# syun88/VLA-from-FastVLM

Measured on AMD Instinct MI355X. Metric: policy steps/sec (img+prompt->action) FastVLM-0.5B bs=64, higher is better.
Workload: dtype bf16; 1 GPU; fastvlm-0.5b select_action: letterbox 336^2->1024^2, FastViT-HD, projector, Qwen2 decoder (text-only, reference-literal: 64-token prompt), last-token pool, action head; batch_per_gpu=64, global_batch=64, seq_len=64, image=336, parallelism=replicas x1 (no collective on the inference path), tower_microbatch=0, stream_overlap=True, llm_precision=split-bf16 (hi+lo) operands, fp32 attention

## Files before the change

include/fastvla_hip_testops.h:

```cpp
#ifndef FASTVLA_HIP_TESTOPS_H
#define FASTVLA_HIP_TESTOPS_H

#include "fastvla_hip.h"

#ifdef __cplusplus
extern "C" {
#endif

enum fv_gemm_epilogue {
  FV_EPI_BIAS = 0,
  FV_EPI_BIAS_GELU = 1,
  FV_EPI_LS_RES = 2,
  FV_EPI_RES_F32 = 3,
  FV_EPI_SWIGLU = 4,
  FV_EPI_F32 = 5,
  FV_EPI_SWIGLU_SPLIT = 7,
  FV_EPI_SWIGLU_F16 = 8,
  FV_EPI_GELU_GRAD = 9,
  FV_EPI_MUL_AUX = 10,
  FV_EPI_F16 = 11,
  FV_EPI_MUL_GELUP = 12
};
int fv_op_gemm(const void* A, int lda, const void* W, int M, int N, int K, const float* bias, const float* scale,
               const void* res, int ldr, void* out, int ldo, int epilogue, fv_stream s);
// ... 14 lines not shown
int fv_op_stem_mfma(const void* pix, const void* wp, const float* bias, void* y, int B, int S, int Cout, fv_stream s);
int fv_op_stem_fused(const void* pix, const void* wp, const float* b1, const float* w2, const float* b2, void* y, int B,
                     int S, int Cout, fv_stream s);
int fv_op_stem_fused_images(const void* img, int dtype, int B, int C, int Hin, int Win, float pad_value, int resize_with_padding, const void* wp,
                            const float* b1, const float* w2, const float* b2, void* y, int S, int Cout, fv_stream s);
int fv_op_layernorm_rows(const void* x, const float* w, const float* b, void* y, int rows, int C, float eps,
                         fv_stream s);
int fv_op_attention(const void* q, const void* k, const void* v, int ldq, int ldk, int ldv, void* out, int ldo, int B,
                    int T, int heads, int kv_heads, int D, int causal, const int32_t* lens, float scale, fv_stream s);
int fv_op_attention_bf16(const void* q, const void* k, const void* v, int ldq, int ldk, int ldv, void* out, int ldo, int B, int T, int heads, int kv_heads, int D,
                         int causal, const int32_t* lens, int len_add, float scale, fv_stream s);
int fv_op_tower_attention_bwd(const void* qkv, int ld, const void* dO, int lddo, void* dqkv, int ldd, float* stats, int B, int T, int heads, float scale, fv_stream s);
int fv_op_rmsnorm(const float* x, const float* w, void* y_bf16, int rows, int H, float eps, fv_stream s);
int fv_op_rope(void* qkv, int ld, int rows, int T, int heads, int kv_heads, int D, float theta, fv_stream s);
int fv_op_attention_bwd(const float* qkv, int ld, const float* dO, float* dqkv, void* out_bf16_scratch, float* stat_scratch, int B, int T,
                        int heads, int kv_heads, int D, const int32_t* lens, float theta, fv_stream s);
int fv_op_attention_bwd_routes(const float* qkv, int ld, const float* dO, int lddo, float* dqkv, void* out_bf16, int ldo, float* stat, float* part, int B, int T,
                               int heads, int kv_heads, int D, const int32_t* lens, int len_add, float theta, int use_split, fv_stream s);
int fv_op_attention_f32(void* qkv, int ld, void* out, int ldo, int B, int T, int heads, int kv_heads, int D, const int32_t* lens, int len_add,
                        const void* rope_table, const void* pre, int ldp, int Np, float* lse, int lo8, int use_split, fv_stream s);
int fv_op_rmsnorm_forms(const float* x, const float* w, void* y, void* y_lo, int ldy, int rows, int H, float eps, int f16, unsigned* sat, int lo8, fv_stream s);
int fv_op_embed_gather(const int32_t* ids, const void* table, const float* img_tokens, float* x, int B, int T, int Ni, int H, int vocab, fv_stream s);
int fv_op_pool_norm(const float* x, const int32_t* lens, const float* w, float* pooled, int B, int Ttot, int Ni, int H, float eps, int mode, fv_stream s);
int fv_op_rmsnorm_bwd(const float* x, const float* w, const float* dy, const float* dres, float* dx, float* dw, float* scratch, int rows,
                      int H, float eps, fv_stream s);

int fv_op_se_gelu(const void* x, const float* w1, const float* b1, const float* w2, const float* b2, void* y,
                  float* scratch, int B, int P, int C, int R, fv_stream s);

int fv_op_dwconv_mfma(const void* x, const void* ttab, const float* bias, void* y, int B, int H, int W, int C, int k, int gelu,
                      fv_stream s);
int fv_op_dwconv_s2_mfma(const void* x, const void* ttab, const float* bias, void* y, int B, int H, int W, int C, int gelu,
                         fv_stream s);
int fv_op_dwconv_pair(const void* x, const void* t3, const float* b3, const void* t7, const float* b7, void* y1, void* y2, int B,
                      int H, int W, int C, fv_stream s);
int fv_op_convffn(const void* x, const void* w1, const float* b1, const void* w2p, const float* b2, const float* ls,
                  const void* res, void* out, int M, int C, fv_stream s);

int fv_op_convffn32(const void* x, const void* wq, const float* b1, const float* b2, const float* ls, const void* res, void* out,
                    int M, int C, fv_stream s);
int fv_op_convffn32_stash(const void* x, const void* wq, const float* b1, const float* b2, const float* ls, const void* res, void* out,
                          int M, int C, void* stash_y, fv_stream s);
int fv_op_gemm_f16_gelup(const void* A, int lda, const void* W, int M, int N, int K, const void* aux, int ldaux, void* out, int ldo, void* h_out, fv_stream s);
int fv_op_dw_wgrad(const void* x, const void* dy, float* dw, float* db, float* scratch, size_t scratch_floats, int B, int H, int W, int C, int k, int stride, int mult, fv_stream s);
int fv_op_dw_dgrad(const void* dy, const float* w, const void* res, void* dx, int B, int Hi, int Wi, int Ci, int k, int stride, int mult, int round_w, unsigned* sat,
                   fv_stream s);
int fv_op_dw_dgrad_mfma(const void* dy, const void* ttab16, const void* res, void* dx, int B, int H, int W, int C, int k, unsigned* sat, fv_stream s);
int fv_op_convffn32_split(const void* x, const void* wq, const float* b1, const float* b2, const float* ls, const void* res, void* out,
                          int M, int C, float* part, size_t part_bytes, fv_stream s);

int fv_op_lora_direct_scratch_floats(int R, int rank, int max_cols, size_t* out_floats);
int fv_op_lora_direct(int kind, int part_mask, int rank, int Np, int K, int qd, int kd, const int64_t* a_off, const int64_t* b_off, const void* dY, const void* X,
                      int xkind, int ldx, int lo_off, int R, const float* lora, float* lora_grads, float scale, float* scratch, size_t scratch_floats, fv_stream s);


int fv_op_chunk_loss(const float* a, const float* t, const uint8_t* pad, float* g, float* partial, size_t partial_floats, float* loss, float* metrics,
                     int64_t n, int A, int kind, float beta, float loss_scale, fv_stream s);

int fv_op_chunk_loss_weighted(const float* a, const float* t, const uint8_t* pad, const float* dim_w, const float* step_w, float* g, float* partial,
                              size_t partial_floats, float* loss, float* metrics, int64_t n, int A, int K, int kind, float beta, float loss_scale, fv_stream s);

int fv_op_head_loss_backward(int feat, int ds, int da, int hid, int fus, int time_dim, const float* P, const float* actions, const float* targets,
                             const uint8_t* pad, int kind, float beta, int chunk, int B, const void* saved, float* loss, float* metrics, float* G,
                             float* scratch, size_t scratch_floats, float* d_pooled, fv_stream s);
int fv_op_head_loss_backward_draws(int feat, int ds, int da, int hid, int fus, int time_dim, int draws, const float* P, const float* actions, const float* targets,
                                   const uint8_t* pad, const float* dim_w, const float* step_w, int kind, float beta, int chunk, int B, const void* saved, float* loss,
// ... 17 lines not shown
```

vla-from-fastvlm_amd/csrc/kernels.h:

```cpp
#pragma once
#include <hip/hip_runtime.h>
#include <stdint.h>

#include "../../include/fastvla_hip.h"
#include "../../include/fastvla_hip_testops.h"
#include "common.h"

namespace fv {

struct GemmArgs {
  const bf16_t* A; int lda;
  const bf16_t* W;
  int M, N, K;
  const float* bias;
  const float* scale;
  const void* res; int ldr;
  void* out; int ldo;
  int epi;
  int ksplit = 0;
  int f16 = 0;
  float* splitk_ws = nullptr;
  size_t splitk_bytes = 0;
  int lo_off = 0;
  int no_tail = 0;
// ... 17 lines not shown
void convffn32_pack(const float* w1, const float* w2, float* out, int C);
int launch_convffn32(const bf16_t* x, const bf16_t* wq, const float* b1, const float* b2, const float* ls,
                     const bf16_t* res, bf16_t* out, int M, int C, int hidden, hipStream_t s, float* part = nullptr, size_t part_bytes = 0,
                     bf16_t* stash_y = nullptr);
bool convffn32_stash_supported(int M, int C);

int launch_letterbox(const void* img, int dtype, int B, int C, int Hin, int Win, int S, float pad_value, int letterbox,
                     bf16_t* pix, hipStream_t s);
int launch_letterbox_norm(const void* img, int dtype, int B, int C, int Hin, int Win, int S, float pad_value, int letterbox, const float* mean3,
                          const float* std3, int range_heuristic, unsigned* vmax_scratch, bf16_t* pix, hipStream_t s);
int launch_augment_draw(const fv_augment_config* cfg, const void* img, int dtype, int B, int C, int Hin, int Win, uint64_t seed, uint64_t offset,
                        uint64_t sample_base, fv_augment_sample* table, hipStream_t s);
int launch_letterbox_augmented(const void* img, int dtype, int B, int C, int Hin, int Win, int S, float pad_value, int letterbox,
                               const fv_augment_sample* table, float value_max, bf16_t* pix, hipStream_t s);
int launch_stem_conv(const bf16_t* pix, const float* w, const float* bias, bf16_t* y, int B, int S, int Cout,
                     hipStream_t s);
void stem_mfma_pack(const float* w27, float* out, int Cout);
int launch_stem_mfma(const bf16_t* pix, const bf16_t* wp, const float* bias, bf16_t* y, int B, int S, int Cout, hipStream_t s);
bool stem_fused_supported(int S, int C0);
int launch_stem_fused(const bf16_t* pix, const bf16_t* wp, const float* b1, const float* w2, const float* b2, bf16_t* y, int B,
                      int S, int C0, hipStream_t s);
int launch_stem_fused_lb(const void* img, int dtype, int B, int C, int Hin, int Win, float pad_value, int letterbox, const bf16_t* wp,
                         const float* b1, const float* w2, const float* b2, bf16_t* y, int S, int C0, hipStream_t s);
int launch_dwconv(const bf16_t* x, const float* w, const float* bias, bf16_t* y, int B, int H, int W, int C, int k,
                  int stride, int mult, int gelu, hipStream_t s);
bool dwconv_mfma_supported(int W, int C, int k, int stride, int mult);
size_t dwconv_toeplitz_elems(int C, int k);
void dwconv_toeplitz_pack(const float* w_tapmajor, float* out, int C, int k);
size_t dwconv_s2_toeplitz_elems(int C);
void dwconv_s2_toeplitz_pack(const float* w_tapmajor, float* out, int C);
bool dwconv_s2_mfma_supported(int H, int W, int C, int k, int stride, int mult);
int launch_dwconv_s2_mfma(const bf16_t* x, const bf16_t* ttab, const float* bias, bf16_t* y, int B, int H, int W, int C, int gelu,
                          hipStream_t s);
bool dwconv_pair_supported(int B, int H, int W, int C);
int launch_dwconv_pair(const bf16_t* x, const bf16_t* t3, const float* b3, const bf16_t* t7, const float* b7, bf16_t* y1, bf16_t* y2,
                       int B, int H, int W, int C, hipStream_t s);
int launch_dwconv_mfma(const bf16_t* x, const bf16_t* ttab, const float* bias, bf16_t* y, int B, int H, int W, int C, int k,
                       int gelu, hipStream_t s);
int launch_layernorm_rows(const bf16_t* x, const float* w, const float* b, bf16_t* y, int rows, int C, float eps,
                          hipStream_t s);
int launch_se_gelu(const bf16_t* x, const float* w1, const float* b1, const float* w2, const float* b2, bf16_t* y,
                   float* scratch, int B, int P, int C, int R, hipStream_t s);
int launch_attention(const bf16_t* q, const bf16_t* k, const bf16_t* v, int ldq, int ldk, int ldv, bf16_t* out,
                     int ldo, int B, int T, int heads, int kv_heads, int D, int causal, const int32_t* lens,
                     int len_add, float scale, hipStream_t s, const unsigned* skip = nullptr);

int launch_embed_gather(const int32_t* ids, const bf16_t* table, const float* img_tokens, float* x, int B, int T,
                        int Ni, int H, int vocab, hipStream_t s, const unsigned* skip = nullptr);
int launch_rmsnorm(const float* x, const float* w, bf16_t* y, bf16_t* y_lo, int ldy, int rows, int H, float eps, hipStream_t s,
                   int f16 = 0, unsigned* sat = nullptr,
                   int lo8 = 0, const unsigned* skip = nullptr);
int launch_bf16_to_f16(bf16_t* p, size_t n, float scale, hipStream_t s, unsigned* maxbits = nullptr);
int launch_bf16_to_w8(const bf16_t* w, void* w8, size_t rows, int K, hipStream_t s, unsigned* maxbits = nullptr);
int launch_rope_f32(float* qkv, const float2* table, int ld, int rows, int T, int heads, int kv_heads, int D, hipStream_t s, const unsigned* skip = nullptr);
int launch_attention_f32(float* qkv, int ld, bf16_t* out_hi, bf16_t* out_lo, int ldo, int B, int T, int heads,
                         int kv_heads, int D, const int32_t* lens, int len_add, float scale, hipStream_t s, const float2* rope = nullptr,
                         const float* pre = nullptr, int ldp = 0, int Np = 0,
                         float* lse = nullptr,
                         int lo8 = 0,
                         void* split_scratch = nullptr,
                         const unsigned* skip = nullptr);
constexpr int FV_ATTN_SPLIT_MIN_T = 128;
int launch_rope(bf16_t* qkv, const float2* table, int ld, int rows, int T, int heads, int kv_heads, int D,
                hipStream_t s, const unsigned* skip = nullptr);
void rope_table_host(float* cos_sin_pairs, int T, int D, float theta);
int launch_pool_norm(const float* x, const int32_t* lens, const float* w, float* pooled, int B, int Ttot, int Ni,
// ... 211 lines not shown
```

vla-from-fastvlm_amd/csrc/ops_api.hip:

```cpp
#include <cmath>
#include <vector>

#include "kernels.h"

extern "C" {

int fv_op_gemm(const void* A, int lda, const void* W, int M, int N, int K, const float* bias, const float* scale,
               const void* res, int ldr, void* out, int ldo, int epilogue, fv_stream s) {
  fv::GemmArgs g{static_cast<const bf16_t*>(A), lda, static_cast<const bf16_t*>(W), M, N, K, bias, scale, res, ldr, out, ldo, epilogue};
  return fv::launch_gemm(g, static_cast<hipStream_t>(s));
}
int fv_op_gemm_ksplit(const void* A, int lda, const void* W, int M, int N, int K, const float* bias, const void* res, int ldr,
                      void* out, int ldo, int epilogue, fv_stream s) {
  fv::GemmArgs g{static_cast<const bf16_t*>(A), lda, static_cast<const bf16_t*>(W), M, N, K, bias, nullptr, res, ldr, out, ldo, epilogue};
  g.ksplit = true;
  return fv::launch_gemm(g, static_cast<hipStream_t>(s));
}
int fv_op_gemm_splitk(const void* A, int lda, const void* W, int M, int N, int K, const float* bias, const void* res, int ldr,
                      void* out, int ldo, int epilogue, int ksplit, void* ws, size_t ws_bytes, fv_stream s) {
  fv::GemmArgs g{static_cast<const bf16_t*>(A), lda, static_cast<const bf16_t*>(W), M, N, K, bias, nullptr, res, ldr, out, ldo, epilogue};
  g.ksplit = ksplit != 0;
  g.splitk_ws = static_cast<float*>(ws);
  g.splitk_bytes = ws_bytes;
  return fv::launch_gemm(g, static_cast<hipStream_t>(s));
// ... 160 lines not shown
}

int fv_op_rmsnorm_forms(const float* x, const float* w, void* y, void* y_lo, int ldy, int rows, int H, float eps, int f16, unsigned* sat, int lo8, fv_stream s) {
  return fv::launch_rmsnorm(x, w, static_cast<bf16_t*>(y), static_cast<bf16_t*>(y_lo), ldy, rows, H, eps, static_cast<hipStream_t>(s), f16, sat, lo8);
}

int fv_op_embed_gather(const int32_t* ids, const void* table, const float* img_tokens, float* x, int B, int T, int Ni, int H, int vocab, fv_stream s) {
  return fv::launch_embed_gather(ids, static_cast<const bf16_t*>(table), img_tokens, x, B, T, Ni, H, vocab, static_cast<hipStream_t>(s));
}

int fv_op_pool_norm(const float* x, const int32_t* lens, const float* w, float* pooled, int B, int Ttot, int Ni, int H, float eps, int mode, fv_stream s) {
  return fv::launch_pool_norm(x, lens, w, pooled, B, Ttot, Ni, H, eps, mode, static_cast<hipStream_t>(s));
}

int fv_op_rmsnorm_bwd(const float* x, const float* w, const float* dy, const float* dres, float* dx, float* dw, float* scratch, int rows,
                      int H, float eps, fv_stream s) {
  return fv::launch_rmsnorm_bwd(x, w, dy, dres, dx, dw, scratch, rows, H, eps, static_cast<hipStream_t>(s));
}

int fv_op_se_gelu(const void* x, const float* w1, const float* b1, const float* w2, const float* b2, void* y,
                  float* scratch, int B, int P, int C, int R, fv_stream s) {
  return fv::launch_se_gelu(static_cast<const bf16_t*>(x), w1, b1, w2, b2, static_cast<bf16_t*>(y), scratch, B, P, C, R, static_cast<hipStream_t>(s));
}

int fv_op_dwconv_mfma(const void* x, const void* ttab, const float* bias, void* y, int B, int H, int W, int C, int k, int gelu,
                      fv_stream s) {
  return fv::launch_dwconv_mfma(static_cast<const bf16_t*>(x), static_cast<const bf16_t*>(ttab), bias, static_cast<bf16_t*>(y), B, H, W, C, k,
                                gelu, static_cast<hipStream_t>(s));
}
int fv_op_dwconv_s2_mfma(const void* x, const void* ttab, const float* bias, void* y, int B, int H, int W, int C, int gelu, fv_stream s) {
  return fv::launch_dwconv_s2_mfma(static_cast<const bf16_t*>(x), static_cast<const bf16_t*>(ttab), bias, static_cast<bf16_t*>(y), B, H, W, C,
                                   gelu, static_cast<hipStream_t>(s));
}
int fv_op_dwconv_pair(const void* x, const void* t3, const float* b3, const void* t7, const float* b7, void* y1, void* y2, int B,
                      int H, int W, int C, fv_stream s) {
  return fv::launch_dwconv_pair(static_cast<const bf16_t*>(x), static_cast<const bf16_t*>(t3), b3, static_cast<const bf16_t*>(t7), b7,
                                static_cast<bf16_t*>(y1), static_cast<bf16_t*>(y2), B, H, W, C, static_cast<hipStream_t>(s));
}

int fv_op_convffn(const void* x, const void* w1, const float* b1, const void* w2p, const float* b2, const float* ls,
                  const void* res, void* out, int M, int C, fv_stream s) {
  return fv::launch_convffn(static_cast<const bf16_t*>(x), static_cast<const bf16_t*>(w1), b1, static_cast<const bf16_t*>(w2p), b2, ls,
                            static_cast<const bf16_t*>(res), static_cast<bf16_t*>(out), M, C, 4 * C, static_cast<hipStream_t>(s));
}

int fv_op_convffn32(const void* x, const void* wq, const float* b1, const float* b2, const float* ls, const void* res, void* out,
                    int M, int C, fv_stream s) {
  return fv::launch_convffn32(static_cast<const bf16_t*>(x), static_cast<const bf16_t*>(wq), b1, b2, ls, static_cast<const bf16_t*>(res),
                              static_cast<bf16_t*>(out), M, C, 4 * C, static_cast<hipStream_t>(s));
}

int fv_op_convffn32_stash(const void* x, const void* wq, const float* b1, const float* b2, const float* ls, const void* res, void* out,
                          int M, int C, void* stash_y, fv_stream s) {
  if (!stash_y) return fv_fail(FV_ERR_ARG, "fv_op_convffn32_stash: null stash");
  return fv::launch_convffn32(static_cast<const bf16_t*>(x), static_cast<const bf16_t*>(wq), b1, b2, ls, static_cast<const bf16_t*>(res),
                              static_cast<bf16_t*>(out), M, C, 4 * C, static_cast<hipStream_t>(s), nullptr, 0, static_cast<bf16_t*>(stash_y));
}
int fv_op_gemm_f16_gelup(const void* A, int lda, const void* W, int M, int N, int K, const void* aux, int ldaux, void* out, int ldo, void* h_out, fv_stream s) {
  fv::GemmArgs g{static_cast<const bf16_t*>(A), lda, static_cast<const bf16_t*>(W), M, N, K, nullptr, nullptr, aux, ldaux, out, ldo, FV_EPI_MUL_GELUP};
  g.f16 = 1;
  g.stash = h_out;
  return fv::launch_gemm(g, static_cast<hipStream_t>(s));
}

int fv_op_dw_wgrad(const void* x, const void* dy, float* dw, float* db, float* scratch, size_t scratch_floats, int B, int H, int W, int C, int k, int stride, int mult, fv_stream s) {
  const int pad = k / 2, Ho = (H + 2 * pad - k) / stride + 1, Wo = (W + 2 * pad - k) / stride + 1;
// ... 142 lines not shown
```

vla-from-fastvlm_amd/csrc/tower_kernels.hip:

```cpp
#include "kernels.h"
#include "letterbox.h"
#include <cstdlib>

namespace fv {
namespace {

__device__ __forceinline__ uint2 lb_pixel(const LbParams& p, int b, int y, int x) {
  float v[3] = {p.pad, p.pad, p.pad};
  const int dx = x - p.pl, dy = y - p.pt;
  if (dx >= 0 && dx < p.rw && dy >= 0 && dy < p.rh) {
    const float sx = lb_src(dx, p.sw);
    const int x0 = min((int)sx, p.Win - 1), x1 = min(x0 + 1, p.Win - 1);
    const float wx = lb_frac(sx, x0);
    const float sy = lb_src(dy, p.sh);
    const int y0 = min((int)sy, p.Hin - 1), y1 = min(y0 + 1, p.Hin - 1);
    const float wy = lb_frac(sy, y0);
    const int nc = p.C >= 3 ? 3 : 1;
    for (int c = 0; c < nc; ++c) {
      const size_t plane = ((size_t)b * p.C + c) * p.Hin * p.Win;
      const float t0 = lb_lerp(lb_fetch(p, plane, y0, x0), lb_fetch(p, plane, y0, x1), wx);
      const float t1 = lb_lerp(lb_fetch(p, plane, y1, x0), lb_fetch(p, plane, y1, x1), wx);
      v[c] = lb_lerp(t0, t1, wy);
    }
    if (nc == 1) v[1] = v[2] = v[0];
// ... 743 lines not shown
        uint2 u;
        u.x = pack_bf2(g[0].x, g[0].y);
        u.y = pack_bf2(g[1].x, g[1].y);
        *reinterpret_cast<uint2*>(sX + ((rg * 4 + jr) * 4 + q) * OC + ((co ^ sig) << 3)) = u;
      }
  }
  __syncthreads();
  {
    const int cg = tid & 7, quad = (tid >> 3) & 3, row = tid >> 5;
    const int sig = (row >> 1) & 1;
    uint2 r[8];
#pragma unroll
    for (int e = 0; e < 8; ++e) r[e] = *reinterpret_cast<const uint2*>(sX + (row * 4 + quad) * OC + (((cg * 8 + e) ^ sig) << 3));
    const int oy = tyb * TH + row, ox0 = tx * TW + quad * 4;
    if (oy < Ho) {
      bf16_t* yp = y + (((size_t)b * Ho + oy) * Wo + ox0) * (2 * C) + 2 * c0 + cg * 8;
#pragma unroll
      for (int j = 0; j < 4; ++j) {
        if (ox0 + j < Wo) {
          uint4 o;
          const uint32_t sel = (j & 1) ? 0x07060302u : 0x05040100u;
#define FV_PX(A, B) __builtin_amdgcn_perm((j & 2) ? r[B].y : r[B].x, (j & 2) ? r[A].y : r[A].x, sel)
          o.x = FV_PX(0, 1); o.y = FV_PX(2, 3); o.z = FV_PX(4, 5); o.w = FV_PX(6, 7);
#undef FV_PX
          *reinterpret_cast<uint4*>(yp + (size_t)j * (2 * C)) = o;
        }
      }
    }
  }
  __syncthreads();
  tx = txn; tyb = tybn; b = bn;
  }
}

#ifndef DW_MARCH_OCC
#define DW_MARCH_OCC 2
#endif
typedef __attribute__((ext_vector_type(4))) _Float16 f16x4_t;
__device__ __forceinline__ _Float16 f2h_ovf(float v) { return (_Float16)(fabsf(v) > FV_F16_MAX ? copysignf(__builtin_inff(), v) : v); }
template <bool GRAD> struct MarchAux { typedef const float* type; };
template <> struct MarchAux<true> { typedef unsigned* type; };
template <bool GRAD> using march_aux_t = typename MarchAux<GRAD>::type;
template <int K, bool GRAD = false>
__global__ __launch_bounds__(256, DW_MARCH_OCC) void dwconv_march_kernel(const bf16_t* __restrict__ x, const bf16_t* __restrict__ ttab,
                                                               march_aux_t<GRAD> __restrict__ aux, bf16_t* __restrict__ y,
                                                               int H, int W, int C, int gelu, int tiles_x, int nslices, const bf16_t* __restrict__ res = nullptr) {
  constexpr int TW = 32, PAD = K / 2, IW = TW + K - 1;
  constexpr int NQ = (IW + 3) / 4, NM = (K + 3 + 3) / 4;
  constexpr int RS = NQ * 256 + 64, RSO = 8 * 256 + 64;
  constexpr int T_BYTES = 2 * K * NM * 512;
#if DW_MARCH_OCC >= 3
  __shared__ __attribute__((aligned(16))) char smem[16 * RS];
#else
  __shared__ __attribute__((aligned(16))) char smem[16 * RS + 8 * RSO];
#endif
  extern __shared__ __attribute__((aligned(16))) char smem_lo[];
  static_assert(!GRAD || DW_MARCH_OCC < 3, "the GRAD instances keep an output tile of their own");
  char* sX = smem;

  const int tid = threadIdx.x, lane = tid & 63, wid = tid >> 6;
  int bid = xcd_remap(blockIdx.x, gridDim.x);
  const int slice = bid % nslices; bid /= nslices;
  const int tx = bid % tiles_x;
  const long b = bid / tiles_x;
  const int c0 = slice * 32;
  const int gg = wid & 1, rg = wid >> 1;
// ... 735 lines not shown
size_t dwconv_toeplitz_elems(int C, int k) { return (size_t)(C / 16) * k * ((k + 6) / 4) * 256; }
void dwconv_toeplitz_pack(const float* w_tapmajor, float* out, int C, int k) {
  const int NM = (k + 6) / 4;
  for (int g = 0; g < C / 16; ++g)
    for (int ky = 0; ky < k; ++ky)
      for (int m = 0; m < NM; ++m)
        for (int bch = 0; bch < 16; ++bch)
          for (int i = 0; i < 4; ++i)
            for (int kk = 0; kk < 4; ++kk) {
              const int kx = 4 * m + kk - i;
              out[((((size_t)(g * k + ky) * NM + m) * 16 + bch) * 4 + i) * 4 + kk] =
                  (kx >= 0 && kx < k) ? w_tapmajor[(size_t)(ky * k + kx) * C + g * 16 + bch] : 0.0f;
            }
}
size_t dwconv_s2_toeplitz_elems(int C) { return (size_t)(C / 16) * 2 * 7 * 4 * 256; }
void dwconv_s2_toeplitz_pack(const float* w_tapmajor, float* out, int C) {
  for (int g = 0; g < C / 16; ++g)
    for (int e = 0; e < 2; ++e)
      for (int ky = 0; ky < 7; ++ky)
        for (int m = 0; m < 4; ++m)
          for (int bch = 0; bch < 16; ++bch)
            for (int i = 0; i < 4; ++i)
              for (int kk = 0; kk < 4; ++kk) {
                const int kx = 4 * m + kk - 2 * i;
                out[(((((size_t)(g * 2 + e) * 7 + ky) * 4 + m) * 16 + bch) * 4 + i) * 4 + kk] =
                    (kx >= 0 && kx < 7) ? w_tapmajor[(size_t)(ky * 7 + kx) * (2 * C) + 2 * (g * 16 + bch) + e] : 0.0f;
              }
}
bool dwconv_s2_mfma_supported(int H, int W, int C, int k, int stride, int mult) {
  return k == 7 && stride == 2 && mult == 2 && C % 32 == 0 && H % 2 == 0 && W % 2 == 0 && W >= 16;
}
int launch_dwconv_s2_mfma(const bf16_t* x, const bf16_t* ttab, const float* bias, bf16_t* y, int B, int H, int W, int C, int gelu,
                          hipStream_t s) {
  if (!x || !ttab || !bias || !y) return fv_fail(FV_ERR_ARG, "dwconv_s2_mfma: null pointer");
  if (B <= 0 || H <= 0 || !dwconv_s2_mfma_supported(H, W, C, 7, 2, 2)) return fv_fail(FV_ERR_UNSUPPORTED, "dwconv_s2_mfma: unsupported shape H=%d W=%d C=%d", H, W, C);
  const int Ho = H / 2, Wo = W / 2;
  const int tiles_x = (Wo + 15) / 16, tiles_y = (Ho + 7) / 8, nsl = C / 32;
  const long nblk = (long)B * tiles_x * tiles_y * nsl;
  if (nblk > 0x7fffffffL) return fv_fail(FV_ERR_ARG, "dwconv_s2_mfma: grid too large");
  static int cus = 0;
  if (!cus) {
    int dev = 0;
    hipDeviceProp_t prop;
    cus = (hipGetDevice(&dev) == hipSuccess && hipGetDeviceProperties(&prop, dev) == hipSuccess && prop.multiProcessorCount > 0) ? prop.multiProcessorCount : 256;
  }
  const long tiles = nblk / nsl, tpx = (tiles + 7) / 8;
  long chains = (2L * cus / 8) / nsl;
  if (chains < 1) chains = 1;
  if (chains > tpx) chains = tpx;
  hipLaunchKernelGGL(dwconv_s2_mfma_kernel, dim3((unsigned)(8 * chains * nsl)), dim3(256), 0, s, x, ttab, bias, y, H, W, C, Ho, Wo, gelu, tiles_x, tiles_y, nsl, B);
  FV_HIP_CHECK(hipGetLastError());
  return FV_OK;
}

bool dwconv_mfma_supported(int W, int C, int k, int stride, int mult) {
  return stride == 1 && mult == 1 && (k == 3 || k == 7) && W >= 16 && C % 32 == 0;
}

int launch_dwconv_mfma(const bf16_t* x, const bf16_t* ttab, const float* bias, bf16_t* y, int B, int H, int W, int C, int k,
                       int gelu, hipStream_t s) {
  if (!x || !ttab || !bias || !y) return fv_fail(FV_ERR_ARG, "dwconv_mfma: null pointer");
  if (B <= 0 || H <= 0 || !dwconv_mfma_supported(W, C, k, 1, 1)) return fv_fail(FV_ERR_UNSUPPORTED, "dwconv_mfma: unsupported shape W=%d C=%d k=%d", W, C, k);
#ifndef DW_TH7
#define DW_TH7 8
#endif
  const int th = (k == 7 && H >= 32) ? DW_TH7 : 8;
  const int tiles_x = (W + 31) / 32, tiles_y = (H + th - 1) / th, nsl = C / 32;
  const long nblk = (long)B * tiles_x * tiles_y * nsl;
  if (nblk > 0x7fffffffL) return fv_fail(FV_ERR_ARG, "dwconv_mfma: grid too large");
#ifndef DW_NO_MARCH
  if (k == 7 && H >= 16) {
    const long nstrips = (long)B * tiles_x * nsl;
// ... 165 lines not shown
```

vla-from-fastvlm_amd/fastvla_hip/_lib.py:

```python
from __future__ import annotations

import ctypes as C
import os
from pathlib import Path

FV_MAX_STAGES = 8
FV_F32, FV_BF16, FV_U8, FV_I32 = 0, 1, 2, 3
EPI_BIAS, EPI_BIAS_GELU, EPI_LS_RES, EPI_RES_F32, EPI_SWIGLU, EPI_F32 = range(6)
EPI_SWIGLU_SPLIT = 7
EPI_SWIGLU_F16 = 8


class FastVLAHipError(RuntimeError):
    status = 0


class ModelDesc(C.Structure):
    _fields_ = [
        ("llm_hidden", C.c_int32), ("llm_layers", C.c_int32), ("llm_heads", C.c_int32), ("llm_kv_heads", C.c_int32),
        ("llm_head_dim", C.c_int32), ("llm_inter", C.c_int32), ("llm_vocab", C.c_int32),
        ("rope_theta", C.c_float), ("rms_eps", C.c_float),
        ("tower_stages", C.c_int32),
        ("tower_layers", C.c_int32 * FV_MAX_STAGES), ("tower_dims", C.c_int32 * FV_MAX_STAGES),
        ("tower_is_attn", C.c_int32 * FV_MAX_STAGES),
# ... 164 lines not shown
    "fv_train_tower_backward": (_i, [_vp, _vp, _vp, _i, _vp, C.c_size_t, _vp, BUCKET_CB, _vp, _vp]),
    "fv_train_tower_read_unit": (_i, [_vp, _i, _i, _vp, C.c_size_t, _vp, _vp]),
    "fv_train_tower_unit": (_i, [_vp, _i, _vp, _vp, _f, _i, _vp, C.c_size_t, _vp, _vp, _vp, _vp]),
    "fv_profile": (_i, [_vp, _i]),
    "fv_profile_read": (_i, [_vp, C.POINTER(ProfileEntry), C.POINTER(GemmProfile), _i, C.POINTER(_i)]),
    "fv_adamw_clip_step": (_i, [_vp, _vp, _vp, _vp, _vp, _i64, C.POINTER(AdamWHParams), _i64, _vp, _vp]),
    "fv_adamw_groups_create": (_i, [_vp, C.POINTER(AdamWGroup), _i, _i64, C.POINTER(_vp)]),
    "fv_adamw_groups_destroy": (_i, [_vp, _vp]),
    "fv_adamw_clip_step_groups": (_i, [_vp, _vp, _vp, _vp, _vp, _i64, C.POINTER(AdamWHParams), _vp, _i64, _vp, _vp, _vp]),
    "fv_adamw_clip_step_ema": (_i, [_vp, _vp, _vp, _vp, _vp, _vp, _f, _i64, C.POINTER(AdamWHParams), _vp, _i64, _vp, _vp, _vp]),
}

OPS_SIGNATURES = {
    "fv_op_gemm": (_i, [_vp, _i, _vp, _i, _i, _i, _vp, _vp, _vp, _i, _vp, _i, _i, _vp]),
    "fv_op_gemm_f16": (_i, [_vp, _i, _vp, _i, _i, _i, _vp, _vp, _i, _vp, _i, _i, _vp, C.c_size_t, _vp]),
    "fv_op_gemm_lo8": (_i, [_vp, _i, _vp, _vp, _i, _i, _i, _vp, _vp, _i, _vp, _i, _i, _vp, C.c_size_t, _vp]),
    "fv_op_lo8_pack": (_i, [_vp, _vp, _i, _vp, _vp, _i, _i, _i, _vp]),
    "fv_op_gemm_ksplit": (_i, [_vp, _i, _vp, _i, _i, _i, _vp, _vp, _i, _vp, _i, _i, _vp]),
    "fv_op_gemm_tn": (_i, [_vp, _i, _vp, _i, _i, _i, _i, _i, _vp, _vp, _i, _vp, C.c_size_t, _vp]),
    "fv_op_gemm_splitk": (_i, [_vp, _i, _vp, _i, _i, _i, _vp, _vp, _i, _vp, _i, _i, _i, _vp, C.c_size_t, _vp]),
    "fv_op_dwconv": (_i, [_vp, _vp, _vp, _vp, _i, _i, _i, _i, _i, _i, _i, _i, _vp]),
    "fv_op_stem_conv": (_i, [_vp, _vp, _vp, _vp, _i, _i, _i, _vp]),
    "fv_op_stem_mfma": (_i, [_vp, _vp, _vp, _vp, _i, _i, _i, _vp]),
    "fv_op_stem_fused": (_i, [_vp, _vp, _vp, _vp, _vp, _vp, _i, _i, _i, _vp]),
    "fv_op_stem_fused_images": (_i, [_vp, _i, _i, _i, _i, _i, _f, _i, _vp, _vp, _vp, _vp, _vp, _i, _i, _vp]),
    "fv_op_layernorm_rows": (_i, [_vp, _vp, _vp, _vp, _i, _i, _f, _vp]),
    "fv_op_attention": (_i, [_vp, _vp, _vp, _i, _i, _i, _vp, _i, _i, _i, _i, _i, _i, _i, _vp, _f, _vp]),
    "fv_op_attention_bf16": (_i, [_vp, _vp, _vp, _i, _i, _i, _vp, _i, _i, _i, _i, _i, _i, _i, _vp, _i, _f, _vp]),
    "fv_op_tower_attention_bwd": (_i, [_vp, _i, _vp, _i, _vp, _i, _vp, _i, _i, _i, _f, _vp]),
    "fv_op_rmsnorm": (_i, [_vp, _vp, _vp, _i, _i, _f, _vp]),
    "fv_op_rope": (_i, [_vp, _i, _i, _i, _i, _i, _i, _f, _vp]),
    "fv_op_dwconv_mfma": (_i, [_vp, _vp, _vp, _vp, _i, _i, _i, _i, _i, _i, _vp]),
    "fv_op_dwconv_s2_mfma": (_i, [_vp, _vp, _vp, _vp, _i, _i, _i, _i, _i, _vp]),
    "fv_op_dwconv_pair": (_i, [_vp, _vp, _vp, _vp, _vp, _vp, _vp, _i, _i, _i, _i, _vp]),
    "fv_op_convffn": (_i, [_vp, _vp, _vp, _vp, _vp, _vp, _vp, _vp, _i, _i, _vp]),
    "fv_op_convffn32": (_i, [_vp, _vp, _vp, _vp, _vp, _vp, _vp, _i, _i, _vp]),
    "fv_op_convffn32_stash": (_i, [_vp, _vp, _vp, _vp, _vp, _vp, _vp, _i, _i, _vp, _vp]),
    "fv_op_gemm_f16_gelup": (_i, [_vp, _i, _vp, _i, _i, _i, _vp, _i, _vp, _i, _vp, _vp]),
    "fv_op_dw_wgrad": (_i, [_vp, _vp, _vp, _vp, _vp, C.c_size_t, _i, _i, _i, _i, _i, _i, _i, _vp]),
    "fv_op_dw_dgrad": (_i, [_vp, _vp, _vp, _vp, _i, _i, _i, _i, _i, _i, _i, _i, _vp, _vp]),
    "fv_op_dw_dgrad_mfma": (_i, [_vp, _vp, _vp, _vp, _i, _i, _i, _i, _i, _vp, _vp]),
    "fv_op_convffn32_split": (_i, [_vp, _vp, _vp, _vp, _vp, _vp, _vp, _i, _i, _vp, C.c_size_t, _vp]),
    "fv_op_lora_direct_scratch_floats": (_i, [_i, _i, _i, C.POINTER(C.c_size_t)]),
    "fv_op_lora_direct": (_i, [_i, _i, _i, _i, _i, _i, _i, _vp, _vp, _vp, _vp, _i, _i, _i, _i, _vp, _vp, _f, _vp, C.c_size_t, _vp]),
    "fv_op_attention_bwd": (_i, [_vp, _i, _vp, _vp, _vp, _vp, _i, _i, _i, _i, _i, _vp, _f, _vp]),
    "fv_op_attention_bwd_routes": (_i, [_vp, _i, _vp, _i, _vp, _vp, _i, _vp, _vp, _i, _i, _i, _i, _i, _vp, _i, _f, _i, _vp]),
    "fv_op_rmsnorm_bwd": (_i, [_vp, _vp, _vp, _vp, _vp, _vp, _vp, _i, _i, _f, _vp]),
    "fv_op_attention_f32": (_i, [_vp, _i, _vp, _i, _i, _i, _i, _i, _i, _vp, _i, _vp, _vp, _i, _i, _vp, _i, _i, _vp]),
    "fv_op_rmsnorm_forms": (_i, [_vp, _vp, _vp, _vp, _i, _i, _i, _f, _i, _vp, _i, _vp]),
    "fv_op_embed_gather": (_i, [_vp, _vp, _vp, _vp, _i, _i, _i, _i, _i, _vp]),
    "fv_op_pool_norm": (_i, [_vp, _vp, _vp, _vp, _i, _i, _i, _i, _f, _i, _vp]),
    "fv_op_chunk_loss": (_i, [_vp, _vp, _vp, _vp, _vp, C.c_size_t, _vp, _vp, _i64, _i, _i, _f, _f, _vp]),
    "fv_op_chunk_loss_weighted": (_i, [_vp, _vp, _vp, _vp, _vp, _vp, _vp, C.c_size_t, _vp, _vp, _i64, _i, _i, _i, _f, _f, _vp]),
    "fv_op_head_loss_backward": (_i, [_i, _i, _i, _i, _i, _i, _vp, _vp, _vp, _vp, _i, _f, _i, _i, _vp, _vp, _vp, _vp, _vp, C.c_size_t, _vp, _vp]),
    "fv_op_head_loss_backward_draws": (_i, [_i, _i, _i, _i, _i, _i, _i, _vp, _vp, _vp, _vp, _vp, _vp, _i, _f, _i, _i, _vp, _vp, _vp, _vp, _vp, C.c_size_t, _vp, _vp]),
    "fv_op_flow_vjp": (_i, [_i, _i, _i, _i, _i, _i, _vp, _vp, _vp, _vp, _i, _vp, _f, _vp, _vp, _vp, _vp, C.c_size_t, _vp]),
    "fv_op_flow_vjp_prefix": (_i, [_i, _i, _i, _i, _i, _i, _i, _vp, _vp, _vp, _vp, _i, _vp, _f, _vp, _vp, _vp, _vp, C.c_size_t, _vp]),
    "fv_op_flow_select": (_i, [_vp, _i, _i, _i, _i, _vp, _i, _vp, _vp, _i, _vp, _vp, _vp, _vp, _vp, _vp, _vp, _vp, _vp]),
    "fv_op_head_saved_cat_offset": (_i, [_i, _i, _i, _i, _i, _i, _i, _i, _i, C.POINTER(C.c_size_t)]),
    "fv_op_se_gelu": (_i, [_vp, _vp, _vp, _vp, _vp, _vp, _vp, _i, _i, _i, _i, _vp]),
}

_LIB = None
_OPS = None


# ... 82 lines not shown
```

Before: 21.85 steps/s.

## Add row-marching stride-2 depthwise conv kernel with LDS ring buffer

Adds a new stride-2 7x7 depthwise MFMA kernel in which each block marches down the full image height for one x-tile and channel slice. Input rows are held in a 21-row LDS ring, and global fetches for the next group are prefetched into registers while the current group computes. By default it replaces the per-tile kernel whenever Ho>=16, and a route argument allows forcing either path. The intent is to stop reloading the halo rows that overlapping tiles share and to overlap loads with compute. The cost is a much smaller grid (no tiles_y dimension) and a large dynamic LDS footprint, which may reduce parallelism.

```diff
diff --git a/include/fastvla_hip_testops.h b/include/fastvla_hip_testops.h
--- a/include/fastvla_hip_testops.h
+++ b/include/fastvla_hip_testops.h
@@ -70,6 +70,8 @@
                       fv_stream s);
 int fv_op_dwconv_s2_mfma(const void* x, const void* ttab, const float* bias, void* y, int B, int H, int W, int C, int gelu,
                          fv_stream s);
+int fv_op_dwconv_s2_route(const void* x, const void* ttab, const float* bias, void* y, int B, int H, int W, int C, int gelu, int route,
+                          fv_stream s);
 int fv_op_dwconv_pair(const void* x, const void* t3, const float* b3, const void* t7, const float* b7, void* y1, void* y2, int B,
                       int H, int W, int C, fv_stream s);
 int fv_op_convffn(const void* x, const void* w1, const float* b1, const void* w2p, const float* b2, const float* ls,
diff --git a/vla-from-fastvlm_amd/csrc/kernels.h b/vla-from-fastvlm_amd/csrc/kernels.h
--- a/vla-from-fastvlm_amd/csrc/kernels.h
+++ b/vla-from-fastvlm_amd/csrc/kernels.h
@@ -73,6 +73,8 @@
 bool dwconv_s2_mfma_supported(int H, int W, int C, int k, int stride, int mult);
 int launch_dwconv_s2_mfma(const bf16_t* x, const bf16_t* ttab, const float* bias, bf16_t* y, int B, int H, int W, int C, int gelu,
                           hipStream_t s);
+int launch_dwconv_s2_mfma_route(const bf16_t* x, const bf16_t* ttab, const float* bias, bf16_t* y, int B, int H, int W, int C, int gelu,
+                                int route, hipStream_t s);
 bool dwconv_pair_supported(int B, int H, int W, int C);
 int launch_dwconv_pair(const bf16_t* x, const bf16_t* t3, const float* b3, const bf16_t* t7, const float* b7, bf16_t* y1, bf16_t* y2,
                        int B, int H, int W, int C, hipStream_t s);
diff --git a/vla-from-fastvlm_amd/csrc/ops_api.hip b/vla-from-fastvlm_amd/csrc/ops_api.hip
--- a/vla-from-fastvlm_amd/csrc/ops_api.hip
+++ b/vla-from-fastvlm_amd/csrc/ops_api.hip
@@ -216,6 +216,10 @@
   return fv::launch_dwconv_s2_mfma(static_cast<const bf16_t*>(x), static_cast<const bf16_t*>(ttab), bias, static_cast<bf16_t*>(y), B, H, W, C,
                                    gelu, static_cast<hipStream_t>(s));
 }
+int fv_op_dwconv_s2_route(const void* x, const void* ttab, const float* bias, void* y, int B, int H, int W, int C, int gelu, int route, fv_stream s) {
+  return fv::launch_dwconv_s2_mfma_route(static_cast<const bf16_t*>(x), static_cast<const bf16_t*>(ttab), bias, static_cast<bf16_t*>(y), B, H, W, C,
+                                         gelu, route, static_cast<hipStream_t>(s));
+}
 int fv_op_dwconv_pair(const void* x, const void* t3, const float* b3, const void* t7, const float* b7, void* y1, void* y2, int B,
                       int H, int W, int C, fv_stream s) {
   return fv::launch_dwconv_pair(static_cast<const bf16_t*>(x), static_cast<const bf16_t*>(t3), b3, static_cast<const bf16_t*>(t7), b7,
diff --git a/vla-from-fastvlm_amd/csrc/tower_kernels.hip b/vla-from-fastvlm_amd/csrc/tower_kernels.hip
--- a/vla-from-fastvlm_amd/csrc/tower_kernels.hip
+++ b/vla-from-fastvlm_amd/csrc/tower_kernels.hip
@@ -799,6 +799,169 @@
   tx = txn; tyb = tybn; b = bn;
   }
 }
+
+__global__ __launch_bounds__(256, 2) void dwconv_s2_march_kernel(const bf16_t* __restrict__ x, const bf16_t* __restrict__ ttab,
+                                                                  const float* __restrict__ bias, bf16_t* __restrict__ y, int H,
+                                                                  int W, int C, int Ho, int Wo, int gelu, int tiles_x, int nslices) {
+  constexpr int K = 7, TW = 16, PAD = 3, IW = 2 * TW + K - 2;
+  constexpr int NQ = (IW + 3) / 4, NM = 4;
+  constexpr int RS = NQ * 256 + 64;
+  constexpr int RING = 21, UR = 16, PR = RING - UR;
+  constexpr int OC = 512 + 16;
+  constexpr int UTASK = UR * NQ * 4, PTASK = PR * NQ * 4, TPT = (UTASK + 255) / 256;
+  extern __shared__ __attribute__((aligned(16))) char smem_s2m[];
+  char* sX = smem_s2m;
+  char* sO = smem_s2m + RING * RS;
+  const int tid = threadIdx.x, lane = tid & 63, wid = tid >> 6;
+  int bid = xcd_remap(blockIdx.x, gridDim.x);
+  const int slice = bid % nslices; bid /= nslices;
+  const int tx = bid % tiles_x;
+  const int b = bid / tiles_x;
+  const int c0 = slice * 32;
+  const int gg = wid & 1, eo = wid >> 1;
+  const int bch = lane >> 2, jr = lane & 3;
+  const int ng = (Ho + 7) >> 3;
+
+  s16x4 afr[K][NM];
+  {
+    const char* tsrc = reinterpret_cast<const char*>(ttab) + (size_t)(slice * 2 + gg) * (2 * K * NM * 512) + (size_t)eo * (K * NM * 512) + lane * 8;
+#pragma unroll
+    for (int ky = 0; ky < K; ++ky)
+#pragma unroll
+      for (int m = 0; m < NM; ++m) afr[ky][m] = __builtin_bit_cast(s16x4, *reinterpret_cast<const uint2*>(tsrc + (ky * NM + m) * 512));
+  }
+  uint4 px[TPT][4];
+  int trow[TPT], tcol[TPT], toff[TPT];
+  uint32_t tcell[TPT];
+#pragma unroll
+  for (int tt = 0; tt < TPT; ++tt) {
+    const int task = min(tid + 256 * tt, UTASK - 1);
+    const int cg = task & 3, quad = (task >> 2) % NQ, row = (task >> 2) / NQ;
+    trow[tt] = row;
+    tcol[tt] = quad * 4;
+    toff[tt] = (row * W + quad * 4) * C + cg * 8;
+    tcell[tt] = (uint32_t)(quad * 256 + cg * 64) | (uint32_t)((((quad & 3) << 1) | (cg >> 1)) << 3);
+  }
+  const int ix0 = 2 * tx * TW - PAD;
+  auto fetch = [&](int r0, int ntask) {
+    const bf16_t* org = x + ((long)b * H * W + (long)r0 * W + ix0) * C + c0;
+#pragma unroll
+    for (int tt = 0; tt < TPT; ++tt) {
+      const bool rok = tid + 256 * tt < ntask && (unsigned)(r0 + trow[tt]) < (unsigned)H;
+#pragma unroll
+      for (int j = 0; j < 4; ++j)
+        px[tt][j] = (rok && (unsigned)(ix0 + tcol[tt] + j) < (unsigned)W) ? *reinterpret_cast<const uint4*>(org + toff[tt] + j * C)
+                                                                         : make_uint4(0, 0, 0, 0);
+    }
+  };
+  auto stage = [&](int p0, int ntask) {
+#pragma unroll
+    for (int tt = 0; tt < TPT; ++tt) {
+      if (tid + 256 * tt < ntask) {
+        const uint32_t d[4][4] = {{px[tt][0].x, px[tt][0].y, px[tt][0].z, px[tt][0].w}, {px[tt][1].x, px[tt][1].y, px[tt][1].z, px[tt][1].w},
+                                  {px[tt][2].x, px[tt][2].y, px[tt][2].z, px[tt][2].w}, {px[tt][3].x, px[tt][3].y, px[tt][3].z, px[tt][3].w}};
+        int pr = p0 + trow[tt];
+        pr -= pr >= RING ? RING : 0;
+        const uint32_t dst = (uint32_t)(pr * RS) + tcell[tt];
+#pragma unroll
+        for (int dd = 0; dd < 4; ++dd) {
+          uint2 ev, od;
+          ev.x = __builtin_amdgcn_perm(d[1][dd], d[0][dd], 0x05040100u);
+          ev.y = __builtin_amdgcn_perm(d[3][dd], d[2][dd], 0x05040100u);
+          od.x = __builtin_amdgcn_perm(d[1][dd], d[0][dd], 0x07060302u);
+          od.y = __builtin_amdgcn_perm(d[3][dd], d[2][dd], 0x07060302u);
+          *reinterpret_cast<uint2*>(sX + (dst ^ (uint32_t)((2 * dd) * 8))) = ev;
+          *reinterpret_cast<uint2*>(sX + (dst ^ (uint32_t)((2 * dd + 1) * 8))) = od;
+        }
+      }
+    }
+  };
+  uint32_t sw[4];
+#pragma unroll
+  for (int v = 0; v < 4; ++v) sw[v] = (uint32_t)(((gg * 16 + bch) ^ ((v << 1) | gg)) << 3);
+  const int co = 2 * (gg * 16 + bch) + eo;
+  const float bv = bias[2 * c0 + co];
+
+  fetch(-PAD, PTASK);
+  stage(0, PTASK);
+  fetch(PR - PAD, UTASK);
+  stage(PR, UTASK);
+  if (ng > 1) fetch(UR + PR - PAD, UTASK);
+  int gb = 0;
+  for (int g = 0; g < ng; ++g) {
+    __syncthreads();
+    f32x4 acc[2][4];
+#pragma unroll
+    for (int rg = 0; rg < 2; ++rg)
+#pragma unroll
+      for (int q = 0; q < 4; ++q) acc[rg][q] = f32x4{0.f, 0.f, 0.f, 0.f};
+    int lb = gb + 2 * jr;
+    lb -= lb >= RING ? RING : 0;
+#pragma unroll
+    for (int ky = 0; ky < K; ++ky)
+#pragma unroll
+      for (int rg = 0; rg < 2; ++rg) {
+        int pr = lb + rg * 8 + ky;
+        pr -= pr >= RING ? RING : 0;
+        const char* rp = sX + pr * RS;
+        s16x4 xq[NQ];
+#pragma unroll
+        for (int t = 0; t < NQ; ++t) xq[t] = __builtin_bit_cast(s16x4, *reinterpret_cast<const uint2*>(rp + sw[t & 3] + t * 256));
+#pragma unroll
+        for (int m = 0; m < NM; ++m)
+#pragma unroll
+          for (int q = 0; q < 4; ++q) acc[rg][q] = __builtin_amdgcn_mfma_f32_4x4x4bf16_1k(afr[ky][m], xq[2 * q + m], acc[rg][q], 0, 0, 0);
+      }
+    __syncthreads();
+    gb += UR;
+    gb -= gb >= RING ? RING : 0;
+    if (g + 1 < ng) {
+      int ub = gb + PR;
+      ub -= ub >= RING ? RING : 0;
+      stage(ub, UTASK);
+    }
+    if (g + 2 < ng) fetch(UR * (g + 2) + PR - PAD, UTASK);
+
+    {
+      const int sig = (jr >> 1) & 1;
+#pragma unroll
+      for (int rg = 0; rg < 2; ++rg)
+#pragma unroll
+        for (int q = 0; q < 4; ++q) {
+          f32x2 gv[2] = {{acc[rg][q][0] + bv, acc[rg][q][1] + bv}, {acc[rg][q][2] + bv, acc[rg][q][3] + bv}};
+          if (gelu) gelu2_n<2>(gv);
+          uint2 u;
+          u.x = pack_bf2(gv[0].x, gv[0].y);
+          u.y = pack_bf2(gv[1].x, gv[1].y);
+          *reinterpret_cast<uint2*>(sO + ((rg * 4 + jr) * 4 + q) * OC + ((co ^ sig) << 3)) = u;
+        }
+    }
+    __syncthreads();
+    {
+      const int cg = tid & 7, quad = (tid >> 3) & 3, row = tid >> 5;
+      const int sig = (row >> 1) & 1;
+      uint2 r[8];
+#pragma unroll
+      for (int e = 0; e < 8; ++e) r[e] = *reinterpret_cast<const uint2*>(sO + (row * 4 + quad) * OC + (((cg * 8 + e) ^ sig) << 3));
+      const int oy = g * 8 + row, ox0 = tx * TW + quad * 4;
+      if (oy < Ho) {
+        bf16_t* yp = y + (((size_t)b * Ho + oy) * Wo + ox0) * (2 * C) + 2 * c0 + cg * 8;
+#pragma unroll
+        for (int j = 0; j < 4; ++j) {
+          if (ox0 + j < Wo) {
+            uint4 o;
+            const uint32_t sel = (j & 1) ? 0x07060302u : 0x05040100u;
+#define FV_PX(A, B) __builtin_amdgcn_perm((j & 2) ? r[B].y : r[B].x, (j & 2) ? r[A].y : r[A].x, sel)
+            o.x = FV_PX(0, 1); o.y = FV_PX(2, 3); o.z = FV_PX(4, 5); o.w = FV_PX(6, 7);
+#undef FV_PX
+            *reinterpret_cast<uint4*>(yp + (size_t)j * (2 * C)) = o;
+          }
+        }
+      }
+    }
+  }
+}
+constexpr int DWS2M_LDS = 21 * (10 * 256 + 64) + 8 * 4 * (512 + 16);
 
 #ifndef DW_MARCH_OCC
 #define DW_MARCH_OCC 2
@@ -1600,12 +1763,24 @@
 }
 int launch_dwconv_s2_mfma(const bf16_t* x, const bf16_t* ttab, const float* bias, bf16_t* y, int B, int H, int W, int C, int gelu,
                           hipStream_t s) {
+  return launch_dwconv_s2_mfma_route(x, ttab, bias, y, B, H, W, C, gelu, 0, s);
+}
+int launch_dwconv_s2_mfma_route(const bf16_t* x, const bf16_t* ttab, const float* bias, bf16_t* y, int B, int H, int W, int C, int gelu,
+                                int route, hipStream_t s) {
   if (!x || !ttab || !bias || !y) return fv_fail(FV_ERR_ARG, "dwconv_s2_mfma: null pointer");
   if (B <= 0 || H <= 0 || !dwconv_s2_mfma_supported(H, W, C, 7, 2, 2)) return fv_fail(FV_ERR_UNSUPPORTED, "dwconv_s2_mfma: unsupported shape H=%d W=%d C=%d", H, W, C);
+  if (route < 0 || route > 2) return fv_fail(FV_ERR_ARG, "dwconv_s2_mfma: route %d not in {0, 1, 2}", route);
   const int Ho = H / 2, Wo = W / 2;
   const int tiles_x = (Wo + 15) / 16, tiles_y = (Ho + 7) / 8, nsl = C / 32;
   const long nblk = (long)B * tiles_x * tiles_y * nsl;
   if (nblk > 0x7fffffffL) return fv_fail(FV_ERR_ARG, "dwconv_s2_mfma: grid too large");
+  if (route == 2 || (route == 0 && Ho >= 16)) {
+    static bool attr = false;
+    if (!attr) { FV_HIP_CHECK(hipFuncSetAttribute(reinterpret_cast<const void*>(&dwconv_s2_march_kernel), hipFuncAttributeMaxDynamicSharedMemorySize, DWS2M_LDS)); attr = true; }
+    hipLaunchKernelGGL(dwconv_s2_march_kernel, dim3((unsigned)((long)B * tiles_x * nsl)), dim3(256), DWS2M_LDS, s, x, ttab, bias, y, H, W, C, Ho, Wo, gelu, tiles_x, nsl);
+    FV_HIP_CHECK(hipGetLastError());
+    return FV_OK;
+  }
   static int cus = 0;
   if (!cus) {
     int dev = 0;
diff --git a/vla-from-fastvlm_amd/fastvla_hip/_lib.py b/vla-from-fastvlm_amd/fastvla_hip/_lib.py
--- a/vla-from-fastvlm_amd/fastvla_hip/_lib.py
+++ b/vla-from-fastvlm_amd/fastvla_hip/_lib.py
@@ -220,6 +220,7 @@
     "fv_op_rope": (_i, [_vp, _i, _i, _i, _i, _i, _i, _f, _vp]),
     "fv_op_dwconv_mfma": (_i, [_vp, _vp, _vp, _vp, _i, _i, _i, _i, _i, _i, _vp]),
     "fv_op_dwconv_s2_mfma": (_i, [_vp, _vp, _vp, _vp, _i, _i, _i, _i, _i, _vp]),
+    "fv_op_dwconv_s2_route": (_i, [_vp, _vp, _vp, _vp, _i, _i, _i, _i, _i, _i, _vp]),
     "fv_op_dwconv_pair": (_i, [_vp, _vp, _vp, _vp, _vp, _vp, _vp, _i, _i, _i, _i, _vp]),
     "fv_op_convffn": (_i, [_vp, _vp, _vp, _vp, _vp, _vp, _vp, _vp, _i, _i, _vp]),
     "fv_op_convffn32": (_i, [_vp, _vp, _vp, _vp, _vp, _vp, _vp, _i, _i, _vp]),
```

Result: no change. 21.94 steps/s (median of 6 runs) (+0.4%).
